# 2Retr0/GodotOceanWaves

Hardware: AMD Instinct MI355X
Metric: displacement+normal maps/sec, 1024^2 x 4 cascades; achieved HBM GB/s vs peak (higher is better)
Workload: dtype f32; 1 GPU; 1024^2 x 4 cascades per GPU, steady-state tick (modulate + 2-D IFFT + unpack/foam), delta=1/50 s, SURVEY 8d cascade table; map_size=1024, cascades_per_gpu=4, parallelism=cascade-sharded x1, gather=none

## Files before the change

### godotoceanwaves_amd/csrc/ow_device.h

```cpp
#pragma once

#include <stdint.h>
#include <math.h>

#if defined(__HIPCC__)
#define OW_DEV __device__ __forceinline__
#define OW_HD __host__ __device__ __forceinline__
#define OW_DEVICE_BUILD 1
#define OW_SCHED_FENCE() __builtin_amdgcn_sched_barrier(0)
#else
#define OW_DEV inline
#define OW_HD inline
#define OW_DEVICE_BUILD 0
#define OW_SCHED_FENCE() ((void)0)
#endif

namespace ow {

#if OW_DEVICE_BUILD
typedef float cplx __attribute__((ext_vector_type(2)));
#else
struct alignas(8) cplx {
    float x, y;
};
// ... 457 lines not shown
    float f;
    __builtin_memcpy(&f, &x, 4);
    return f;
#endif
}
OW_DEV uint32_t f2h2(float lo, float hi) {
#if OW_DEVICE_BUILD && OW_CVT_PK
    uint32_t r;
    asm("v_cvt_pk_f16_f32 %0, %1, %2" : "=v"(r) : "v"(lo), "v"(hi));
    return r;
#else
    return (uint32_t)f2h(lo) | ((uint32_t)f2h(hi) << 16);
#endif
}

struct CascadeFrame {
    float tile_x, tile_y;
    float time;
    float whitecap;
    float foam_grow_rate;
    float foam_decay;
    int32_t cascade;
    int32_t fault;
};
constexpr uint32_t kStatusRowSyncTimeout = 1u;
constexpr unsigned long long kRowSyncTimeoutTicks = 2000000ull;
constexpr int plan_lp_rows(int N) { return 128 / plan_T(N) > 0 ? 128 / plan_T(N) : 1; }
constexpr int plan_lp_threads(int N) { return plan_lp_rows(N) * kLayers * plan_T(N); }
constexpr int plan_lp_lds_cplx(int N) { return plan_region_cplx(N) * plan_lp_rows(N) * kLayers + plan_tw_total(N); }
constexpr int plan_lp_handoff_cplx(int N) { return plan_lp_threads(N) / 2; }

template <int N>
struct TickPlan {
    static constexpr int Q = plan_lp_threads(N) / plan_wg_threads(N);
    static constexpr int GPS = N / kWgRows;
    static_assert(Q >= 1 && plan_lp_threads(N) % plan_wg_threads(N) == 0 && (GPS / 2) % Q == 0, "block shapes of the two passes must nest");
    static constexpr int full(int slots) { return slots * GPS / Q; }
    static constexpr int upper(int slots) { return slots * (GPS / 2) / Q; }
    static constexpr int row0(int slots) { return (slots * 3 + Q - 1) / Q; }
    static constexpr int items_1(int slots) { return 2 * full(slots) + upper(slots) + row0(slots); }
    static constexpr int items_1_compact(int slots) { return full(slots); }
    static OW_HD void decode_compact(int item, int sub, int &slot, int &row0) {
        const int group = item * Q + sub;
        slot = group / GPS;
        row0 = (group % GPS) * kWgRows;
    }
    static constexpr int items_2(int slots) { return slots * (N / plan_lp_rows(N)); }
    static constexpr int kPipeRows = plan_lp_rows(N) / 2 > 0 ? plan_lp_rows(N) / 2 : 1;
    static constexpr int items_2_pipe(int slots) { return slots * (N / kPipeRows); }
    static OW_HD bool decode(int item, int sub, int slots, int &L, int &slot, int &row0) {
        const int n_full = full(slots), n_upper = upper(slots);
        if (item < 2 * n_full) {
            L = item < n_full ? 0 : 2;
            const int group = (item < n_full ? item : item - n_full) * Q + sub;
            slot = group / GPS;
            row0 = (group % GPS) * kWgRows;
            return true;
        }
        if (item < 2 * n_full + n_upper) {
            L = 1;
            const int group = (item - 2 * n_full) * Q + sub;
            slot = group / (GPS / 2);
            row0 = N / 2 + (group % (GPS / 2)) * kWgRows;
            return true;
        }
        const int r = (item - 2 * n_full - n_upper) * Q + sub;
        const bool active = r < slots * 3;
        slot = active ? r / 3 : 0;
        L = 3 + (active ? r % 3 : 0);
        row0 = 0;
        return active;
    }
};

constexpr int kMaxTickGroup = 16;
struct TickGroupArgs {
    float time1[kMaxTickGroup][8];
    int32_t tbase2[kMaxTickGroup];
    int32_t tbase1[kMaxTickGroup];
    int32_t slots, n2, n1, d2, d1;
    int32_t pair_compact;
    int32_t first2, slots2;
    int32_t first1, slots1;
    int32_t step1;
    int32_t p2_pipe;
    int32_t p1_compact;
};
struct PairFrame {
    float tile_x, tile_y, whitecap, foam_grow_rate, foam_decay;
    int32_t cascade;
};
struct PairArgs {
    PairFrame c[8];
    float time1[8];
    int32_t tbase2, tbase1;
    int32_t n2, n1;
    int32_t first2, first1;
    int32_t fault, pad;
};
OW_HD CascadeFrame pair_frame(const PairArgs &g, int launch_slot) {
    const PairFrame &f = g.c[launch_slot];
    CascadeFrame cf;
    cf.tile_x = f.tile_x, cf.tile_y = f.tile_y, cf.time = g.time1[launch_slot], cf.whitecap = f.whitecap;
    cf.foam_grow_rate = f.foam_grow_rate, cf.foam_decay = f.foam_decay, cf.cascade = f.cascade, cf.fault = g.fault;
    return cf;
}
constexpr int32_t kFaultRowSync = 1;
constexpr int kMaxCascades = 8;
struct FrameArgs {
    CascadeFrame c[kMaxCascades];
};

#if OW_DEVICE_BUILD
typedef uint32_t u32x4_t __attribute__((ext_vector_type(4)));
typedef uint32_t u32x2_t __attribute__((ext_vector_type(2)));
struct GBuf {
    __amdgpu_buffer_rsrc_t r;
};
OW_DEV GBuf make_gbuf(const void *base, uint32_t bytes) {
    return GBuf{__builtin_amdgcn_make_buffer_rsrc(const_cast<void *>(base), 0, (int)bytes, 0x00020000)};
}
template <int AUX = 0>
OW_DEV f32x4 gload16(GBuf b, uint32_t voff, uint32_t soff) {
    return __builtin_bit_cast(f32x4, __builtin_amdgcn_raw_buffer_load_b128(b.r, (int)voff, (int)soff, AUX));
}
template <int AUX = 0>
OW_DEV cplx gload8(GBuf b, uint32_t voff, uint32_t soff) {
    return __builtin_bit_cast(cplx, __builtin_amdgcn_raw_buffer_load_b64(b.r, (int)voff, (int)soff, AUX));
}
template <int AUX = 0>
OW_DEV float gload4(GBuf b, uint32_t voff, uint32_t soff) {
    return __builtin_bit_cast(float, __builtin_amdgcn_raw_buffer_load_b32(b.r, (int)voff, (int)soff, AUX));
}
template <int AUX = 0>
OW_DEV uint16_t gload2(GBuf b, uint32_t voff, uint32_t soff) {
    return (uint16_t)__builtin_amdgcn_raw_buffer_load_b16(b.r, (int)voff, (int)soff, AUX);
}
template <int AUX = 0>
OW_DEV void gstore8(GBuf b, uint32_t voff, uint32_t soff, cplx v) {
    __builtin_amdgcn_raw_buffer_store_b64(__builtin_bit_cast(u32x2_t, v), b.r, (int)voff, (int)soff, AUX);
}
template <int AUX = 0>
OW_DEV void gstore8h(GBuf b, uint32_t voff, uint32_t soff, u16x4 v) {
    __builtin_amdgcn_raw_buffer_store_b64(__builtin_bit_cast(u32x2_t, v), b.r, (int)voff, (int)soff, AUX);
}
template <int AUX = 0>
OW_DEV void gstore8w(GBuf b, uint32_t voff, uint32_t soff, uint32_t w0, uint32_t w1) {
    __builtin_amdgcn_raw_buffer_store_b64(u32x2_t{w0, w1}, b.r, (int)voff, (int)soff, AUX);
}
template <int AUX = 0>
OW_DEV void gstore16(GBuf b, uint32_t voff, uint32_t soff, f32x4 v) {
    __builtin_amdgcn_raw_buffer_store_b128(__builtin_bit_cast(u32x4_t, v), b.r, (int)voff, (int)soff, AUX);
}
#else
struct GBuf {
    char *p;
};
OW_DEV GBuf make_gbuf(const void *base, uint32_t) { return GBuf{(char *)const_cast<void *>(base)}; }
template <int AUX = 0>
OW_DEV f32x4 gload16(GBuf b, uint32_t voff, uint32_t soff) { f32x4 v; __builtin_memcpy(&v, b.p + voff + soff, 16); return v; }
template <int AUX = 0>
OW_DEV cplx gload8(GBuf b, uint32_t voff, uint32_t soff) { cplx v; __builtin_memcpy(&v, b.p + voff + soff, 8); return v; }
template <int AUX = 0>
OW_DEV float gload4(GBuf b, uint32_t voff, uint32_t soff) { float v; __builtin_memcpy(&v, b.p + voff + soff, 4); return v; }
template <int AUX = 0>
OW_DEV uint16_t gload2(GBuf b, uint32_t voff, uint32_t soff) { uint16_t v; __builtin_memcpy(&v, b.p + voff + soff, 2); return v; }
template <int AUX = 0>
OW_DEV void gstore8(GBuf b, uint32_t voff, uint32_t soff, cplx v) { __builtin_memcpy(b.p + voff + soff, &v, 8); }
template <int AUX = 0>
OW_DEV void gstore8h(GBuf b, uint32_t voff, uint32_t soff, u16x4 v) { __builtin_memcpy(b.p + voff + soff, &v, 8); }
template <int AUX = 0>
OW_DEV void gstore8w(GBuf b, uint32_t voff, uint32_t soff, uint32_t w0, uint32_t w1) {
    const uint32_t w[2] = {w0, w1};
    __builtin_memcpy(b.p + voff + soff, w, 8);
}
template <int AUX = 0>
OW_DEV void gstore16(GBuf b, uint32_t voff, uint32_t soff, f32x4 v) { __builtin_memcpy(b.p + voff + soff, &v, 16); }
#endif
constexpr int kAuxDefault = 0, kAuxNT = 2, kAuxAgent = 16;

OW_HD constexpr uint32_t t_unit(int n, int layer, int xp, int y) {
    return ((((uint32_t)layer * (uint32_t)(n >> 4) + (uint32_t)(y >> 4)) * (uint32_t)n + (uint32_t)xp) << 4) + (uint32_t)(y & 15);
}
constexpr uint32_t t_cascade_bytes(int n) { return (uint32_t)n * (uint32_t)n * kLayers * 8u; }

OW_DEV float modulate_kcomp(int id, int n, float tile) {
    return ((((float)id - (float)n * 0.5f) * 2.0f) * kPi) / tile;
}

#ifndef OW_OMEGA_ONE_LOAD
#define OW_OMEGA_ONE_LOAD 1
#endif
template <int N>
struct Pass1 {
    static constexpr int T = plan_T(N), P = kP;

    static constexpr int rot(int j) { return (j + 8) & 15; }

    template <int AUX = 0, int J0 = 0, int J1 = P>
    static OW_DEV void load_raw(cplx *a, cplx *b, float *om, int t, int y, GBuf h0_c, GBuf om_c) {
        const int ym = (N - y) % N;
        const int tm = (T - t) % T;
        const uint32_t a_off = (uint32_t)(y * N + t) * 8u;
        const uint32_t b_off = (uint32_t)(ym * N + tm) * 8u;
        const bool lane0 = (t == 0);
        const bool om_mirror = y > N / 2;
        const uint32_t o_off = (om_mirror ? (uint32_t)(ym * N + tm) : (uint32_t)(y * N + t)) * 4u;
#pragma unroll
        for (int j = J0; j < J1; ++j) {
            const int blk = rot(j);
            a[j] = gload8<AUX>(h0_c, a_off, (uint32_t)(T * blk) * 8u);
            const uint32_t mb = (uint32_t)(T * (15 - blk)), mb0 = (uint32_t)(T * ((16 - blk) % 16));
            constexpr bool one_load = OW_OMEGA_ONE_LOAD && T >= 64;
            if (blk == 0) {
                b[j] = gload8<AUX>(h0_c, lane0 ? b_off : b_off + mb * 8u, 0u);
                if constexpr (one_load) om[j] = gload4<AUX>(om_c, (om_mirror && !lane0) ? o_off + mb * 4u : o_off, 0u);
                else om[j] = om_mirror ? gload4<AUX>(om_c, lane0 ? o_off : o_off + mb * 4u, 0u) : gload4<AUX>(om_c, o_off, 0u);
            } else {
                b[j] = gload8<AUX>(h0_c, lane0 ? b_off + (uint32_t)T * 8u : b_off, mb * 8u);
                (void)mb0;
                if constexpr (one_load) {
#if OW_DEVICE_BUILD
                    const bool mirror_u = __builtin_amdgcn_readfirstlane((int)om_mirror) != 0;
#else
                    const bool mirror_u = om_mirror;
#endif
                    om[j] = gload4<AUX>(om_c, (om_mirror && lane0) ? o_off + (uint32_t)T * 4u : o_off, mirror_u ? mb * 4u : (uint32_t)(T * blk) * 4u);
                } else {
                    om[j] = om_mirror ? gload4<AUX>(om_c, lane0 ? o_off + (uint32_t)T * 4u : o_off, mb * 4u)
                                      : gload4<AUX>(om_c, o_off, (uint32_t)(T * blk) * 4u);
                }
            }
        }
    }
    static constexpr bool kPairwise = N >= 1024;
#ifndef OW_P1_PAIRWISE
#define OW_P1_PAIRWISE 7
#endif
    template <int J0 = 0, int J1 = P>
    static OW_DEV void modulate(cplx *h, const cplx *a, const cplx *b, const float *om, float time) {
        static_assert(J0 % 2 == 0 && J1 % 2 == 0, "texels are modulated two at a time");
#if OW_DEVICE_BUILD && (OW_P1_PAIRWISE & 1)
        if constexpr (kPairwise) {
#pragma unroll
            for (int j = J0; j < J1; j += 2) {
                const cplx ph = cplx{om[j], om[j + 1]} * cplx{time, time};
                const cplx q = ph * cplx{0.318309886183790672f, 0.318309886183790672f};
                const cplx n = cplx{__builtin_rintf(q.x), __builtin_rintf(q.y)};
                cplx r = __builtin_elementwise_fma(-n, cplx{3.140625f, 3.140625f}, ph);
                r = __builtin_elementwise_fma(-n, cplx{9.67502593994140625e-4f, 9.67502593994140625e-4f}, r);
                r = __builtin_elementwise_fma(-n, cplx{1.509957990978376432e-7f, 1.509957990978376432e-7f}, r);
                const cplx z = r * r;
                cplx ps = cplx{2.6343420813645935e-06f, 2.6343420813645935e-06f};
                ps = __builtin_elementwise_fma(ps, z, cplx{-0.00019822614558506757f, -0.00019822614558506757f});
                ps = __builtin_elementwise_fma(ps, z, cplx{0.008333241567015648f, 0.008333241567015648f});
                ps = __builtin_elementwise_fma(ps, z, cplx{-0.1666666567325592f, -0.1666666567325592f});
                const cplx sn = __builtin_elementwise_fma(ps * z, r, r);
                cplx pc = cplx{-2.654252000411361e-07f, -2.654252000411361e-07f};
                pc = __builtin_elementwise_fma(pc, z, cplx{2.478597525623627e-05f, 2.478597525623627e-05f});
                pc = __builtin_elementwise_fma(pc, z, cplx{-0.0013888811226934195f, -0.0013888811226934195f});
                pc = __builtin_elementwise_fma(pc, z, cplx{0.0416666679084301f, 0.0416666679084301f});
                const cplx cs = __builtin_elementwise_fma(pc * z, z, __builtin_elementwise_fma(cplx{-0.5f, -0.5f}, z, cplx{1.0f, 1.0f}));
#pragma unroll
                for (int e = 0; e < 2; ++e) {
                    const uint32_t flip = (uint32_t)(int)(e ? n.y : n.x) << 31;
                    const float se = e ? sn.y : sn.x, ce = e ? cs.y : cs.x;
                    const float s = __builtin_bit_cast(float, __builtin_bit_cast(uint32_t, se) ^ flip);
                    const float c = __builtin_bit_cast(float, __builtin_bit_cast(uint32_t, ce) ^ flip);
                    const cplx pp = cadd(a[j + e], b[j + e]), qq = csub(a[j + e], b[j + e]);
                    h[j + e] = cplx{__builtin_fmaf(pp.x, c, -mul_rn(pp.y, s)), __builtin_fmaf(qq.y, c, mul_rn(qq.x, s))};
                    opaque_inplace(h[j + e]);
                }
                if (j % 4 == 2) OW_SCHED_FENCE();
            }
            return;
        }
#endif
#pragma unroll
        for (int j = J0; j < J1; ++j) {
            const cplx m = expi_phase(mul_rn(om[j], time));
            const cplx pp = cadd(a[j], b[j]), qq = csub(a[j], b[j]);
#if OW_DEVICE_BUILD
            const cplx t1 = pp * m, t2 = qq * m.yx;
#else
            const cplx t1 = cplx{pp.x * m.x, pp.y * m.y}, t2 = cplx{qq.x * m.y, qq.y * m.x};
#endif
            h[j] = cplx{t1.x - t1.y, t2.x + t2.y};
            opaque_inplace(h[j]);
            if (j % 4 == 3) OW_SCHED_FENCE();
        }
    }
    template <int AUX = 0>
    static OW_DEV void load_modulate(cplx *h, int t, int y, GBuf h0_c, GBuf om_c, float time) {
        cplx a[P], b[P];
        float om[P];
        load_raw<AUX>(a, b, om, t, y, h0_c, om_c);
        modulate(h, a, b, om, time);
    }

    static OW_DEV float kx_of(int j, float kx0, float dkx) { return __builtin_fmaf((float)(T * rot(j)), dkx, kx0); }
    static OW_DEV void wave_numbers(float *ik, int t, float ky, float dkx) {
        const float kx0 = (float)(t - N / 2) * dkx, ky2 = __builtin_fmaf(ky, ky, 1e-30f);
#if OW_DEVICE_BUILD && (OW_P1_PAIRWISE & 2)
        if constexpr (kPairwise) {
#pragma unroll
            for (int j = 0; j < P; j += 2) {
// ... 97 lines not shown
    }
    template <int Q>
    static OW_DEV void row0_input(cplx *d, const cplx *h, const float *ik, int t, float ky, float dkx) {
        const float kx0 = (float)(t - N / 2) * dkx;
#pragma unroll
        for (int j = 0; j < P; ++j) {
            const cplx ih = cmuli(h[j]);
            const float kx = kx_of(j, kx0, dkx), ux = kx * ik[j], uy = ky * ik[j];
            const bool corner = (j == kColSlot) && (t == 0);
            float a = 0.0f, b = 0.0f;
            if (Q == 1) { a = corner ? kx - ky * uy : -(ky * uy); b = corner ? ux : 0.0f; }
            if (Q == 2) { a = -ky; b = corner ? -(ky * ux) : ux; }
            if (Q == 3) { a = corner ? 0.0f : ky * ux; b = corner ? -(kx * ux) : __builtin_fmaf(-kx, ux, kx); }
            d[j] = cadd(cscale(h[j], a), cscale(ih, b));
            opaque_inplace(d[j]);
            if (j % 4 == 3) OW_SCHED_FENCE();
        }
    }

    static OW_DEV void stage_write(const cplx *d, int t, cplx *lds_row) {
#pragma unroll
        for (int o = 0; o < P; ++o) lds_row[t + T * o] = d[OutMap<N>::slot_of(o)];
    }
    template <int AUX>
    static OW_DEV void stage_store(int tau, int layer, int row0, const cplx *lds_block, GBuf T_c) {
        const int q = tau % kWgRows, xi = tau / kWgRows;
        const cplx *st = lds_block + q * plan_region_cplx(N);
        const uint32_t voff = t_unit(N, 0, xi, row0 + q) * 8u;
        cplx v[P];
#pragma unroll
        for (int k = 0; k < P; ++k) v[k] = lds_read(st + xi + T * k);
#pragma unroll
        for (int k = 0; k < P; ++k) gstore8<AUX>(T_c, voff, (t_unit(N, layer, 0, 0) + t_unit(N, 0, T * k, 0)) * 8u, v[k]);
    }
    template <int AUX>
    static OW_DEV void stage_store_chunk(int tau, int layer, int row0, const cplx *lds_block, GBuf T_c, int g) {
        const int q = tau % kWgRows, xi = tau / kWgRows;
        const cplx *st = lds_block + q * plan_region_cplx(N);
        const uint32_t voff = t_unit(N, 0, xi, row0 + q) * 8u;
        cplx v[4];
#pragma unroll
        for (int k = 0; k < 4; ++k) v[k] = lds_read(st + xi + T * (4 * g + k));
#pragma unroll
        for (int k = 0; k < 4; ++k) gstore8<AUX>(T_c, voff, (t_unit(N, layer, 0, 0) + t_unit(N, 0, T * (4 * g + k), 0)) * 8u, v[k]);
    }
};

template <int N>
struct Pass2 {
    static constexpr int T = plan_T(N), P = kP;

    static OW_DEV uint32_t t_voff(int t, int xp) {
        return (T >= 16 ? t_unit(N, 0, xp, t) : t_unit(N, 0, xp, 0) + (uint32_t)t) * 8u;
    }
    static constexpr uint32_t t_soff(int layer, int j) {
        return (t_unit(N, layer, 0, 0) + (T >= 16 ? t_unit(N, 0, 0, T * j) : t_unit(N, 0, 0, 16 * (j / 2)) + 8u * (j % 2))) * 8u;
    }
    static constexpr int rot(int j) { return (j + 8) & 15; }
    template <int AUX>
    static OW_DEV void load_layer(cplx *d, int t, int xp, int layer, GBuf T_c) {
        const uint32_t voff = t_voff(t, xp);
#pragma unroll
        for (int j = 0; j < P; ++j) d[j] = gload8<AUX>(T_c, voff, t_soff(layer, rot(j)));
    }
    OW_HD static constexpr uint32_t foam_index(int xp, int yp) { return (uint32_t)xp * N + (uint32_t)(yp % T) * 16u + (uint32_t)(yp / T); }
    static OW_DEV void load_foam(uint32_t *pk, int t, int xp, GBuf foam_c) {
        const uint32_t voff = foam_index(xp, t) * 2u;
        const f32x4 a = gload16(foam_c, voff, 0u), b = gload16(foam_c, voff, 16u);
        const float v[8] = {a.x, a.y, a.z, a.w, b.x, b.y, b.z, b.w};
#pragma unroll
        for (int i = 0; i < 8; ++i) pk[i] = __builtin_bit_cast(uint32_t, v[i]);
    }
    static OW_DEV void store_foam(const uint32_t *pk, int t, int xp, GBuf foam_c) {
        const uint32_t voff = foam_index(xp, t) * 2u;
        float v[8];
#pragma unroll
        for (int i = 0; i < 8; ++i) v[i] = __builtin_bit_cast(float, pk[i]);
        gstore16(foam_c, voff, 0u, f32x4{v[0], v[1], v[2], v[3]});
        gstore16(foam_c, voff, 16u, f32x4{v[4], v[5], v[6], v[7]});
    }

    static OW_DEV void f32_put(GBuf f32_c, uint32_t tex, int o, int ch, float v) {
#if OW_DEVICE_BUILD
        __builtin_amdgcn_raw_buffer_store_b32(__builtin_bit_cast(uint32_t, v), f32_c.r, (int)(tex * 32u + (uint32_t)ch * 4u), (int)((uint32_t)(T * o) * 32u), 0);
#else
        __builtin_memcpy(f32_c.p + tex * 32u + (uint32_t)ch * 4u + (uint32_t)(T * o) * 32u, &v, 4);
#endif
    }

    template <bool F32>
    static OW_DEV void after_layer3(const cplx *l3, const cplx *l2, uint32_t *foam_pk, uint32_t *gy_foam,
                                    uint32_t tex, const CascadeFrame &cf, GBuf f32_c) {
#pragma unroll
        for (int o = 0; o < P; ++o) {
            const int sl = OutMap<N>::slot_of(o);
            const float dhy_dz = l2[sl].x, dhx_dx = l2[sl].y;
            const float dhz_dz = l3[sl].x, dhz_dx = l3[sl].y;
            const float jac = (1.0f + dhx_dx) * (1.0f + dhz_dz) - dhz_dx * dhz_dx;
            const float foam_factor = -fminf(0.0f, jac - cf.whitecap);
            float foam = h2f((uint16_t)((foam_pk[o / 2] >> (16 * (o & 1))) & 0xFFFFu));
            foam = mul_rn(foam, cf.foam_decay);
            foam = foam + mul_rn(foam_factor, cf.foam_grow_rate);
            foam = fminf(fmaxf(foam, 0.0f), 1.0f);
            const float gy = dhy_dz * fast_rcp(1.0f + fabsf(dhz_dz));
            const uint32_t foam_h = f2h(foam);
            gy_foam[o] = (uint32_t)f2h(gy) | (foam_h << 16);
            foam_pk[o / 2] = (o & 1) ? ((foam_pk[o / 2] & 0xFFFFu) | (foam_h << 16)) : ((foam_pk[o / 2] & 0xFFFF0000u) | foam_h);
            if (F32) {
                f32_put(f32_c, tex, o, 4, gy);
                f32_put(f32_c, tex, o, 6, foam);
                f32_put(f32_c, tex, o, 7, jac);
            }
        }
    }
    template <bool F32, int AUX>
    static OW_DEV void after_layer1(const cplx *l1, const float *dhx_dx, const uint32_t *gy_foam, uint32_t tex, GBuf norm_c,
                                    GBuf f32_c) {
#pragma unroll
        for (int o = 0; o < P; ++o) {
            const int sl = OutMap<N>::slot_of(o);
            const float gx = l1[sl].y * fast_rcp(1.0f + fabsf(dhx_dx[o]));
            gstore8h<AUX>(norm_c, tex * 8u, (uint32_t)(T * o) * 8u,
                          u16x4{f2h(gx), (uint16_t)(gy_foam[o] & 0xFFFFu), f2h(dhx_dx[o]), (uint16_t)(gy_foam[o] >> 16)});
            if (F32) {
                f32_put(f32_c, tex, o, 3, gx);
                f32_put(f32_c, tex, o, 5, dhx_dx[o]);
            }
        }
    }
    static constexpr int kRow0Slot = 8;
    static OW_DEV float ky_of(int j, int t, float dky) { return (float)(t + T * (rot(j) - 8)) * dky; }
    OW_HD static constexpr uint32_t pcol_index(int y) { return (uint32_t)(y % T) * 16u + (uint32_t)(y / T); }
    template <int AUX = 0>
    static OW_DEV void derive_dx(cplx *d, int t, int xp, float dky, GBuf pcol_c) {
        const float s = (xp & 1) ? -1.0f : 1.0f;
#pragma unroll
        for (int half = 0; half < 2; ++half) {
            cplx p[P / 2];
#pragma unroll
            for (int i = 0; i < P / 4; ++i) {
                const f32x4 v = gload16<AUX>(pcol_c, (uint32_t)t * 128u, 16u * (uint32_t)(i + (P / 4) * (1 - half)));
                p[2 * i] = cplx{v.x, v.y};
                p[2 * i + 1] = cplx{v.z, v.w};
            }
#pragma unroll
            for (int k = 0; k < P / 2; ++k) {
                const int j = 8 * half + k;
                const float ky = ky_of(j, t, dky);
                d[j] = cplx{__builtin_fmaf(-ky, d[j].y, s * p[k].x), __builtin_fmaf(ky, d[j].x, s * p[k].y)};
            }
            OW_SCHED_FENCE();
        }
    }
    template <int AUX>
    static OW_DEV void load_c1(cplx *d, int t, int xp, float dky, GBuf T_c) {
        static_assert(T >= 16, "the mirrored offsets below assume that T is a multiple of the 16-row line");
        const uint32_t voff = t_voff(t, xp);
        const uint32_t voff_m = t_unit(N, 0, xp, N - t - 7 * T) * 8u;
        const float kyb = (float)t * dky;
        cplx v[P];
#pragma unroll
        for (int j = 0; j < P; ++j)
            v[j] = j < P / 2 ? gload8<AUX>(T_c, voff, t_soff(1, rot(j))) : gload8<AUX>(T_c, voff_m, (t_unit(N, 1, 0, 0) + t_unit(N, 0, 0, T * (15 - j))) * 8u);
        OW_SCHED_FENCE();
#pragma unroll
        for (int j = 0; j < P; ++j) {
            const float sc = 1.0f - __builtin_fmaf((float)(T * (rot(j) - 8)), dky, kyb);
            d[j] = j < P / 2 ? cscale(v[j], sc) : cplx{v[j].x * sc, v[j].y * -sc};
        }
    }
    static OW_DEV void put_row0(cplx *d, int t, cplx r) {
        d[kRow0Slot] = cplx{t == 0 ? r.x : d[kRow0Slot].x, t == 0 ? r.y : d[kRow0Slot].y};
    }
    template <bool F32>
    static OW_DEV void after_f2(const cplx *f2, uint32_t *hz_pk, float *c2, uint32_t tex, GBuf f32_c) {
#pragma unroll
        for (int o = 0; o < P; o += 2) {
            const int sl = OutMap<N>::slot_of(o), sl1 = OutMap<N>::slot_of(o + 1);
            c2[o] = f2[sl].y * f2[sl].y;
            c2[o + 1] = f2[sl1].y * f2[sl1].y;
            hz_pk[o / 2] = (uint32_t)opaque((int)f2h2(f2[sl].x, f2[sl1].x));
            if (F32) {
                f32_put(f32_c, tex, o, 2, f2[sl].x);
                f32_put(f32_c, tex, o + 1, 2, f2[sl1].x);
            }
        }
    }
    template <bool F32, int AUX>
    static OW_DEV void after_f0(const cplx *f0, const uint32_t *hz_pk, int t, int xp, uint32_t tex, GBuf disp_c, GBuf f32_c) {
        const uint32_t w = (uint32_t)((xp ^ t) & 1) << 31;
#pragma unroll
        for (int o = 0; o < P; ++o) {
            const int sl = OutMap<N>::slot_of(o);
            const uint32_t hz_h = (hz_pk[o / 2] >> (16 * (o & 1))) & 0xFFFFu;
            gstore8w<AUX>(disp_c, tex * 8u, (uint32_t)(T * o) * 8u, f2h2(f0[sl].x, f0[sl].y), hz_h | w);
            if (F32) {
                f32_put(f32_c, tex, o, 0, f0[sl].x);
                f32_put(f32_c, tex, o, 1, f0[sl].y);
            }
        }
    }
    template <bool F32>
    static OW_DEV void after_f1(const cplx *f1, float *dhx_dx, uint32_t *gx_pk, uint32_t tex, GBuf f32_c) {
#pragma unroll
        for (int o = 0; o < P; o += 2) {
            const int sl = OutMap<N>::slot_of(o), sl1 = OutMap<N>::slot_of(o + 1);
            dhx_dx[o] = f1[sl].x;
            dhx_dx[o + 1] = f1[sl1].x;
            const float gx = f1[sl].y * fast_rcp(1.0f + fabsf(dhx_dx[o])), gx1 = f1[sl1].y * fast_rcp(1.0f + fabsf(dhx_dx[o + 1]));
            gx_pk[o / 2] = (uint32_t)opaque((int)f2h2(gx, gx1));
            if (F32) {
                f32_put(f32_c, tex, o, 3, gx);
                f32_put(f32_c, tex, o, 5, dhx_dx[o]);
                f32_put(f32_c, tex, o + 1, 3, gx1);
                f32_put(f32_c, tex, o + 1, 5, dhx_dx[o + 1]);
            }
        }
    }
    template <bool F32, int AUX>
    static OW_DEV void after_f3(const cplx *f3, const float *dhx_dx, const float *c2, const uint32_t *gx_pk, uint32_t *foam_pk,
                                uint32_t tex, const CascadeFrame &cf, GBuf norm_c, GBuf f32_c) {
#pragma unroll
        for (int o = 0; o < P; o += 2) {
            float foam[2], gy[2];
#pragma unroll
            for (int e = 0; e < 2; ++e) {
                const int sl = OutMap<N>::slot_of(o + e);
                const float dhy_dz = f3[sl].x, dhz_dz = f3[sl].y;
                const float jac = (1.0f + dhx_dx[o + e]) * (1.0f + dhz_dz) - c2[o + e];
                const float foam_factor = -fminf(0.0f, jac - cf.whitecap);
                float fm = h2f((uint16_t)((foam_pk[o / 2] >> (16 * e)) & 0xFFFFu));
                fm = mul_rn(fm, cf.foam_decay);
                fm = fm + mul_rn(foam_factor, cf.foam_grow_rate);
                foam[e] = fminf(fmaxf(fm, 0.0f), 1.0f);
                gy[e] = dhy_dz * fast_rcp(1.0f + fabsf(dhz_dz));
                if (F32) {
                    f32_put(f32_c, tex, o + e, 4, gy[e]);
                    f32_put(f32_c, tex, o + e, 6, foam[e]);
                    f32_put(f32_c, tex, o + e, 7, jac);
                }
            }
            foam_pk[o / 2] = f2h2(foam[0], foam[1]);
            const uint32_t gy_pk = f2h2(gy[0], gy[1]), gxw = gx_pk[o / 2];
            gstore8w<AUX>(norm_c, tex * 8u, (uint32_t)(T * o) * 8u, (gxw & 0xFFFFu) | (gy_pk << 16), f2h2(dhx_dx[o], foam[0]));
            gstore8w<AUX>(norm_c, tex * 8u, (uint32_t)(T * (o + 1)) * 8u, (gxw >> 16) | (gy_pk & 0xFFFF0000u), f2h2(dhx_dx[o + 1], foam[1]));
        }
    }

    template <bool F32, int AUX>
    static OW_DEV uint16_t unpack_texel(cplx l0, cplx l1, cplx l2, cplx l3, uint16_t foam_prev, int t, int xp, int o, uint32_t tex,
                                        const CascadeFrame &cf, GBuf disp_c, GBuf norm_c, GBuf f32_c) {
        const float dhy_dz = l2.x, dhx_dx = l2.y, dhz_dz = l3.x, dhz_dx = l3.y;
        const float jac = (1.0f + dhx_dx) * (1.0f + dhz_dz) - dhz_dx * dhz_dx;
        const float foam_factor = -fminf(0.0f, jac - cf.whitecap);
        float foam = h2f(foam_prev);
        foam = mul_rn(foam, cf.foam_decay);
        foam = foam + mul_rn(foam_factor, cf.foam_grow_rate);
        foam = fminf(fmaxf(foam, 0.0f), 1.0f);
        const float gy = dhy_dz * fast_rcp(1.0f + fabsf(dhz_dz));
        const float gx = l1.y * fast_rcp(1.0f + fabsf(dhx_dx));
        const uint32_t n1 = f2h2(dhx_dx, foam);
        const uint16_t foam_h = (uint16_t)(n1 >> 16);
        const uint32_t w = (uint32_t)((xp ^ t) & 1) << 31;
        gstore8w<AUX>(norm_c, tex * 8u, (uint32_t)(T * o) * 8u, f2h2(gx, gy), n1);
        gstore8w<AUX>(disp_c, tex * 8u, (uint32_t)(T * o) * 8u, f2h2(l0.x, l0.y), (uint32_t)f2h(l1.x) | w);
        if (F32) {
            f32_put(f32_c, tex, o, 0, l0.x);
            f32_put(f32_c, tex, o, 1, l0.y);
            f32_put(f32_c, tex, o, 2, l1.x);
            f32_put(f32_c, tex, o, 3, gx);
            f32_put(f32_c, tex, o, 4, gy);
            f32_put(f32_c, tex, o, 5, dhx_dx);
            f32_put(f32_c, tex, o, 6, foam);
            f32_put(f32_c, tex, o, 7, jac);
        }
        return foam_h;
    }

    template <bool F32, int AUX>
    static OW_DEV void after_layer0(const cplx *l0, const float *hz, int t, int xp, uint32_t tex, GBuf disp_c, GBuf f32_c) {
        const uint16_t w = (uint16_t)(((xp ^ t) & 1) << 15);
#pragma unroll
        for (int o = 0; o < P; ++o) {
            const int sl = OutMap<N>::slot_of(o);
            gstore8h<AUX>(disp_c, tex * 8u, (uint32_t)(T * o) * 8u, u16x4{f2h(l0[sl].x), f2h(l0[sl].y), f2h(hz[o]), w});
            if (F32) {
                f32_put(f32_c, tex, o, 0, l0[sl].x);
                f32_put(f32_c, tex, o, 1, l0[sl].y);
                f32_put(f32_c, tex, o, 2, hz[o]);
            }
        }
    }
};

struct SpectrumPC {
    int32_t seed_x, seed_y;
    float tile_x, tile_y;
    float alpha, peak_frequency, wind_speed, angle, depth, swell, detail, spread;
};

OW_DEV float omega_texel(int x, int y, int n, float tile_x, float tile_y, float depth) {
#if defined(__clang__)
#pragma clang fp contract(off)
#endif
    const float kx = modulate_kcomp(x, n, tile_x), ky = modulate_kcomp(y, n, tile_y);
    const float k = sqrtf(kx * kx + ky * ky) + 1e-6f;
    const float a = k * depth;
    const float b = a > 9.1f ? 1.0f : (float)tanh((double)a);
    return sqrtf(kG * k * b);
}

OW_DEV void hash_uniform(uint32_t x, uint32_t y, float &u1, float &u2) {
    uint32_t h32 = y + 374761393u + x * 3266489917u;
    h32 = 2246822519u * (h32 ^ (h32 >> 15));
    h32 = 3266489917u * (h32 ^ (h32 >> 13));
    const uint32_t n = h32 ^ (h32 >> 16), n2 = n * 48271u;
    const float rden = 1.0f / 2147483648.0f;
    u1 = (float)((n >> 1) & 0x7FFFFFFFu) * rden;
    u2 = (float)((n2 >> 1) & 0x7FFFFFFFu) * rden;
}

OW_DEV cplx spectrum_amplitude(int idx, int idy, int n, const SpectrumPC &pc) {
#if defined(__clang__)
#pragma clang fp contract(off)
#endif
    const float dkx = (2.0f * kPi) / pc.tile_x, dky = (2.0f * kPi) / pc.tile_y;
// ... 99 lines not shown
```

### godotoceanwaves_amd/csrc/ow_frame_kernels.h

```cpp
#pragma once
#include <type_traits>

#include "ow_kernels.h"

#ifndef OW_P1_WAVES
#define OW_P1_WAVES 4
#endif
namespace ow {

struct Stamp {
    unsigned long long t[16];
    unsigned xcc, pad;
    unsigned long long rt0, rt1;
};
struct DebugArgs {
    Stamp *stamps;
    int never_true;
};

__device__ __forceinline__ void wave_sync() {
    __builtin_amdgcn_fence(__ATOMIC_RELEASE, "wavefront");
    __builtin_amdgcn_wave_barrier();
    __builtin_amdgcn_fence(__ATOMIC_ACQUIRE, "wavefront");
}
// ... 409 lines not shown
    }
    {
        cplx l0[P];
        fetch(l0, 0);
        if constexpr (kFft) row_ifft<N>(l0, t, lds_row, tw_lds, rs);
        OW_STAMP(3, l0[0].x)
        if (kStore || dbg.never_true) {
            Pass2<N>::template after_layer0<F32, AUX_O>(l0, hz, t, xp, tex, disp_c, f32_c);
        } else {
#pragma unroll
            for (int j = 0; j < P; ++j) keep += l0[j].x + l0[j].y + hz[j];
        }
    }
    if (!kStore && keep == 12345.678f) buf.disp[t] = u16x4{1, 2, 3, 4};
    if constexpr ((VAR & 8) != 0) {
        asm volatile("s_waitcnt vmcnt(0)" ::: "memory");
        ts[14] = __builtin_readcyclecounter();
        write_stamps<(plan_wg_threads(N) + 63) / 64>(ts, dbg);
    }
}


template <int N, int AUX_T, int AUX_H, class Issued, class Stamper>
__device__ __forceinline__ void pass1c_item(const DeviceBuffers &buf, const CascadeFrame &cf, float time, int tslot, int row0, int tau, cplx *tw_lds,
                                            cplx *rows_lds, RowSync<N> &rs, Issued issued, Stamper stamp) {
    constexpr int Tn = plan_T(N), P = kP, LC = Pass1<N>::kCompactLayers;
    const int rw = (Tn >= 64) ? __builtin_amdgcn_readfirstlane(tau / Tn) : tau / Tn, t = tau % Tn;
    const uint32_t plane = (uint32_t)N * N;
    cplx *lds_row = rows_lds + rw * plan_region_cplx(N);
    const int y = row0 + rw;
    const GBuf h0_c = make_gbuf(buf.h0 + (size_t)cf.cascade * plane, plane * 8u);
    const GBuf om_c = make_gbuf(buf.omega + (size_t)cf.cascade * plane, plane * 4u);
    const GBuf T_c = make_gbuf(buf.T + (size_t)tslot * plane * kLayers, t_cascade_bytes(N));
    const GBuf pcol_c = make_gbuf(buf.pcol + (size_t)tslot * N, (uint32_t)N * 8u);
    const GBuf rrow_c = make_gbuf(buf.rrow + (size_t)tslot * N * 4, (uint32_t)N * 32u);

    cplx h[P];
    const float dkx = (2.0f * kPi) / cf.tile_x, dky = (2.0f * kPi) / cf.tile_y;
    const float ky = (float)(y - N / 2) * dky;
    float ik[P];
    {
        cplx a[P], b[P];
        float om[P];
        Pass1<N>::template load_raw<AUX_H>(a, b, om, t, y, h0_c, om_c);
        issued();
        Pass1<N>::modulate(h, a, b, om, time);
    }
    stamp(1, h[0].x);
    Pass1<N>::wave_numbers(ik, t, ky, dkx);
    if (t == 0) gstore8(pcol_c, Pass2<N>::pcol_index(y) * 8u, 0u, Pass1<N>::column_term(h, ik, t, dkx));

    if (__builtin_amdgcn_readfirstlane(y) == 0) {
#pragma unroll
        for (int Q = 1; Q <= 3; ++Q) {
            cplx d[P];
            OW_SCHED_FENCE();
            {
                const float kyo = opaque(ky), dkxo = opaque(dkx);
                const int to = opaque(t);
#pragma unroll
                for (int j = 0; j < P; ++j) opaque_inplace(h[j]);
                if (Q == 1) Pass1<N>::template row0_input<1>(d, h, ik, to, kyo, dkxo);
                if (Q == 2) Pass1<N>::template row0_input<2>(d, h, ik, to, kyo, dkxo);
                if (Q == 3) Pass1<N>::template row0_input<3>(d, h, ik, to, kyo, dkxo);
            }
            OW_SCHED_FENCE();
            row_ifft<N, false>(d, t, lds_row, tw_lds, rs);
            rs.sync();
            if (y == 0) {
#pragma unroll
                for (int o = 0; o < P; ++o) gstore8(rrow_c, (uint32_t)(t + Tn * o) * 32u, (uint32_t)Q * 8u, d[OutMap<N>::slot_of(o)]);
            }
        }
    }

    const bool lower = row0 < N / 2;
#pragma unroll
    for (int L = 0; L < LC; ++L) {
        if (L == 1 && lower) continue;
        cplx d[P];
        OW_SCHED_FENCE();
        {
            const float kyo = opaque(ky), dkxo = opaque(dkx);
            const int to = opaque(t);
#pragma unroll
            for (int j = 0; j < P; ++j) opaque_inplace(h[j]);
            auto drain = [&](int g) {
                if (L > 0) Pass1<N>::template stage_store_chunk<AUX_T>(tau, (L == 2 && lower) ? 0 : L - 1, row0, rows_lds, T_c, g);
            };
            if (L == 0) Pass1<N>::template layer_input_c<0>(d, h, ik, to, kyo, dkxo, drain);
            if (L == 1) Pass1<N>::template layer_input_c<1>(d, h, ik, to, kyo, dkxo, drain);
            if (L == 2) Pass1<N>::template layer_input_c<2>(d, h, ik, to, kyo, dkxo, drain);
        }
        OW_SCHED_FENCE();
        stamp(2 + 3 * L, d[0].x);
        if (L > 0) row_ifft<N, true>(d, t, lds_row, tw_lds, rs);
        else row_ifft<N, false>(d, t, lds_row, tw_lds, rs);
        stamp(3 + 3 * L, d[0].x);
        rs.sync();
        Pass1<N>::stage_write(d, t, lds_row);
        lds_barrier();
        if (L == LC - 1) Pass1<N>::template stage_store<AUX_T>(tau, L, row0, rows_lds, T_c);
        stamp(4 + 3 * L, d[0].x);
    }
}

template <int N, int AUX_T = kAuxDefault, int AUX_H = kAuxDefault, bool STAMPS = false>
__global__ __launch_bounds__(plan_wg_threads(N), OW_P1_WAVES) void k_pass1c(DeviceBuffers buf, FrameArgs args, Stamp *stamps = nullptr) {
    unsigned long long ts[STAMPS ? 16 : 1] = {0};
    auto stamp = [&](int k, float keep) {
        if constexpr (STAMPS) {
            asm volatile("" ::"v"(keep));
            ts[k] = __builtin_readcyclecounter();
        }
    };
    stamp(0, 0.0f);
    constexpr int Tn = plan_T(N);
    static_assert(Tn >= 16, "Pass2::load_c1 needs N/16 to be a multiple of the 16-row line");
    __shared__ __attribute__((aligned(16))) cplx lds[plan_wg_lds_cplx(N) + plan_sync_flag_cplx(N, kWgRows)];
    cplx *tw_lds = lds;
    cplx *rows_lds = lds + plan_tw_total(N);
    const int tau = threadIdx.x;
    int *sync_flags = reinterpret_cast<int *>(lds + plan_wg_lds_cplx(N));
    RowSync<N> rs;
    rs.attach(sync_flags, tau / Tn, (tau / 64) & 1);
    rs.watch(buf.status, args.c[0].fault);
    init_row_sync<N>(sync_flags, kWgRows);

    int slot, row0;
    p1_block_to_rows<N>(slot, row0);
    const CascadeFrame cf = args.c[slot];
    fetch_arguments(buf, cf);
    TwPrefetch<N> twp;
    tw_fetch<N>(twp, buf.tw);
    pass1c_item<N, AUX_T, AUX_H>(buf, cf, cf.time, slot, row0, tau, tw_lds, rows_lds, rs, [&] { tw_commit<N>(twp, tw_lds); }, stamp);
    if constexpr (STAMPS) {
        asm volatile("s_waitcnt vmcnt(0)" ::: "memory");
        ts[14] = __builtin_readcyclecounter();
        ts[15] = (unsigned long long)row0;
        if ((threadIdx.x & 63) == 0) {
            Stamp st;
            for (int k = 0; k < 16; ++k) st.t[k] = ts[k];
            st.xcc = xcc_id();
            st.pad = 0;
            stamps[blockIdx.x * ((plan_wg_threads(N) + 63) / 64) + threadIdx.x / 64] = st;
        }
    }
}

constexpr bool p2c_half_table(int N) { return plan_row_spans_waves(N); }
constexpr int p2c_table_total(int N) { return p2c_half_table(N) ? plan_twh_total(N) : plan_tw_total(N); }
template <int N>
__device__ __forceinline__ const cplx *p2c_table(const DeviceBuffers &buf) { return p2c_half_table(N) ? buf.tw_half : buf.tw; }
template <int N, bool F32, int AUX_T, int AUX_O, class RS, class Issued>
__device__ __forceinline__ void pass2c_item(const DeviceBuffers &buf, const CascadeFrame &cf, int tslot, int row0, int tau, cplx *tw_lds, cplx *rows_lds,
                                            RS &rs, Issued issued, uint32_t (&foam_pk)[kP / 2], int foam_io = 3) {
    constexpr int Tn = plan_T(N), P = kP;
    constexpr bool TWH = p2c_half_table(N);
    const int rw = (Tn >= 64) ? __builtin_amdgcn_readfirstlane(tau / Tn) : tau / Tn, t = tau % Tn;
    const uint32_t plane = (uint32_t)N * N;
    cplx *lds_row = rows_lds + rw * plan_region_cplx(N);
    const int xp = row0 + rw;
    const GBuf T_c = make_gbuf(buf.T + (size_t)tslot * plane * kLayers, t_cascade_bytes(N));
    const GBuf pcol_c = make_gbuf(buf.pcol + (size_t)tslot * N, (uint32_t)N * 8u);
    const GBuf rrow_c = make_gbuf(buf.rrow + (size_t)tslot * N * 4, (uint32_t)N * 32u);
    const GBuf disp_c = make_gbuf(buf.disp + (size_t)cf.cascade * plane, plane * 8u);
    const GBuf norm_c = make_gbuf(buf.norm + (size_t)cf.cascade * plane, plane * 8u);
    const GBuf foam_c = make_gbuf(buf.foam + (size_t)cf.cascade * plane, plane * 2u);
    const GBuf f32_c = make_gbuf(F32 ? buf.f32 + (size_t)cf.cascade * plane * 8 : nullptr, F32 ? plane * 32u : 0u);
    const float dky = (2.0f * kPi) / cf.tile_y;
    auto side_row = [&](int q) { return gload8(rrow_c, (uint32_t)xp * 32u, (uint32_t)q * 8u); };

    uint32_t hz_pk[P / 2];
    float c2[P];
    {
        cplx f2[P];
        OW_SCHED_FENCE();
        Pass2<N>::template load_c1<AUX_T>(f2, t, xp, dky, T_c);
        const cplx r2 = side_row(2);
        issued();
        Pass2<N>::put_row0(f2, t, r2);
        row_ifft<N, false, TWH>(f2, opaque(t), lds_row, tw_lds, rs);
        OW_SCHED_FENCE();
        Pass2<N>::template after_f2<F32>(f2, hz_pk, c2, (uint32_t)(xp * N + opaque(t)), f32_c);
    }
    cplx c0[P];
    {
        cplx f0[P];
        OW_SCHED_FENCE();
        const int tq = opaque(t);
        Pass2<N>::template load_layer<AUX_T>(c0, tq, xp, 0, T_c);
#pragma unroll
        for (int j = 0; j < P; ++j) f0[j] = c0[j];
        row_ifft<N, false, TWH>(f0, opaque(t), lds_row, tw_lds, rs);
        OW_SCHED_FENCE();
        const int tr = opaque(t);
        Pass2<N>::template after_f0<F32, AUX_O>(f0, hz_pk, tr, xp, (uint32_t)(xp * N + tr), disp_c, f32_c);
    }
    float dhx_dx[P];
    uint32_t gx_pk[P / 2];
    {
        OW_SCHED_FENCE();
        const int tq = opaque(t);
        Pass2<N>::derive_dx(c0, tq, xp, dky, pcol_c);
        Pass2<N>::put_row0(c0, tq, side_row(1));
        row_ifft<N, false, TWH>(c0, opaque(t), lds_row, tw_lds, rs);
        OW_SCHED_FENCE();
        Pass2<N>::template after_f1<F32>(c0, dhx_dx, gx_pk, (uint32_t)(xp * N + opaque(t)), f32_c);
    }
    {
        cplx f3[P];
        OW_SCHED_FENCE();
        const int tq = opaque(t);
        Pass2<N>::template load_layer<AUX_T>(f3, tq, xp, 2, T_c);
        Pass2<N>::put_row0(f3, tq, side_row(3));
        if (foam_io & 1) Pass2<N>::load_foam(foam_pk, tq, xp, foam_c);
        row_ifft<N, false, TWH>(f3, opaque(t), lds_row, tw_lds, rs);
        OW_SCHED_FENCE();
        const int tr = opaque(t);
        Pass2<N>::template after_f3<F32, AUX_O>(f3, dhx_dx, c2, gx_pk, foam_pk, (uint32_t)(xp * N + tr), cf, norm_c, f32_c);
        if (foam_io & 2) Pass2<N>::store_foam(foam_pk, tr, xp, foam_c);
    }
}

template <int N, bool F32, int AUX_T = kAuxDefault, int AUX_O = kAuxDefault>
__global__ __launch_bounds__(plan_wg_threads(N), 4) void k_pass2c(DeviceBuffers buf, FrameArgs args) {
    constexpr int Tn = plan_T(N);
    static_assert(Tn >= 16, "Pass2::load_c1 needs N/16 to be a multiple of the 16-row line");
    constexpr int TW = p2c_table_total(N), ROWS_CPLX = plan_region_cplx(N) * kWgRows;
    __shared__ __attribute__((aligned(16))) cplx lds[TW + ROWS_CPLX + plan_sync_flag_cplx(N, kWgRows)];
    cplx *tw_lds = lds;
    cplx *rows_lds = lds + TW;
    const int tau = threadIdx.x;
    int *sync_flags = reinterpret_cast<int *>(lds + TW + ROWS_CPLX);
    RowSync<N> rs;
    rs.attach(sync_flags, tau / Tn, (tau / 64) & 1);
    rs.watch(buf.status, args.c[0].fault);
    init_row_sync<N>(sync_flags, kWgRows);

    int slot, row0;
    p2_block_to_rows<N>(slot, row0);
    const CascadeFrame cf = args.c[slot];
    fetch_arguments(buf, cf);
    TablePrefetch<TW, plan_wg_threads(N)> twp;
    twp.fetch(p2c_table<N>(buf));
    uint32_t foam_pk[kP / 2];
    pass2c_item<N, F32, AUX_T, AUX_O>(buf, cf, slot, row0, tau, tw_lds, rows_lds, rs, [&] { twp.commit(tw_lds); }, foam_pk);
}

#ifndef OW_SPLIT_P1_ROWS
#define OW_SPLIT_P1_ROWS 4
#endif
template <int N, int ROWS = kWgRows>
struct SplitGeo {
    static constexpr int H = N / 2, TH = plan_T(H), R = plan_region_cplx(H), TW = plan_tw_total(H);
    static constexpr int kRows = ROWS;
    static constexpr int kThreads = 2 * ROWS * TH;
    static constexpr int kLdsCplx = TW + 2 * ROWS * R;
    static constexpr int kTwPerThread = (TW + kThreads - 1) / kThreads;
};
template <class SG>
struct SplitTw {
    cplx v[SG::kTwPerThread];
};
template <class SG>
__device__ __forceinline__ void split_tw_fetch(SplitTw<SG> &p, const cplx *__restrict__ tw_split, int tau) {
#pragma unroll
    for (int k = 0; k < SG::kTwPerThread; ++k) {
        const int i = tau + k * SG::kThreads;
        p.v[k] = tw_split[i < SG::TW ? i : 0];
    }
}
template <class SG>
__device__ __forceinline__ void split_tw_commit(const SplitTw<SG> &p, cplx *tw_lds, int tau) {
#pragma unroll
    for (int k = 0; k < SG::kTwPerThread; ++k) {
        const int i = tau + k * SG::kThreads;
        if (i < SG::TW) tw_lds[i] = p.v[k];
    }
    lds_barrier();
}

template <int N, int ROWS, int AUX_T, int AUX_H, class Stamper>
__device__ __forceinline__ void pass1c_split_item(const DeviceBuffers &buf, const CascadeFrame &cf, float time, int tslot, int row0, int fault, cplx *tw_lds,
                                                  cplx *rows_lds, int *sync_flags, int tau, Stamper stamp) {
    using SG = SplitGeo<N, ROWS>;
    constexpr int H = SG::H, TH = SG::TH, P = kP, LC = Pass1<N>::kCompactLayers, T = plan_T(N);
    const int wv = __builtin_amdgcn_readfirstlane(tau / 64), rw = wv >> 1, w = wv & 1;
    const int tp = tau % 64, t = 2 * tp + w;
    cplx *vrow = rows_lds + (w * ROWS + rw) * SG::R;
    const uint32_t plane = (uint32_t)N * N;
    RowSync<H> rs;
    RowSync<N> pair;
    pair.attach(sync_flags, rw, w);
    pair.watch(buf.status, fault);
    if (tau < 2 * ROWS) sync_flags[tau] = 0;

    const int y = row0 + rw;
    const GBuf h0_c = make_gbuf(buf.h0 + (size_t)cf.cascade * plane, plane * 8u);
    const GBuf om_c = make_gbuf(buf.omega + (size_t)cf.cascade * plane, plane * 4u);
    const GBuf T_c = make_gbuf(buf.T + (size_t)tslot * plane * kLayers, t_cascade_bytes(N));
    const GBuf pcol_c = make_gbuf(buf.pcol + (size_t)tslot * N, (uint32_t)N * 8u);
    const GBuf rrow_c = make_gbuf(buf.rrow + (size_t)tslot * N * 4, (uint32_t)N * 32u);

    const int q = tau % ROWS, xi = tau / ROWS;
    cplx h[P];
    cplx wxi;
    const float dkx = (2.0f * kPi) / cf.tile_x, dky = (2.0f * kPi) / cf.tile_y;
    const float ky = (float)(y - N / 2) * dky;
    float ik[P];
    {
        SplitTw<SG> twv;
        split_tw_fetch<SG>(twv, buf.tw_split, tau);
        wxi = buf.tw_split[SG::TW + xi];
        cplx a[P], b[P];
        float om[P];
        Pass1<N>::template load_raw<AUX_H>(a, b, om, t, y, h0_c, om_c);
        stamp(1, 0.0f);
        split_tw_commit<SG>(twv, tw_lds, tau);
        stamp(2, a[15].x + om[15]);
        Pass1<N>::modulate(h, a, b, om, time);
    }
    stamp(3, h[15].x);
    Pass1<N>::wave_numbers(ik, t, ky, dkx);
    if (t == 0) gstore8(pcol_c, Pass2<N>::pcol_index(y) * 8u, 0u, Pass1<N>::column_term(h, ik, t, dkx));

    const cplx *e_reg = rows_lds + q * SG::R, *o_reg = rows_lds + (ROWS + q) * SG::R;
    auto combine = [&](int m, cplx &lo, cplx &hi) {
        const cplx e = lds_read(e_reg + xi + T * m), o = lds_read(o_reg + xi + T * m);
        cplx wx = wxi;
        opaque_inplace(wx);
        cplx tw = wx;
        switch (m) {
            case 1: tw = cmul_const(wx, root32_cos(2), root32_sin(2)); break;
            case 2: tw = cmul_const(wx, root32_cos(4), root32_sin(4)); break;
            case 3: tw = cmul_const(wx, root32_cos(6), root32_sin(6)); break;
            case 4: tw = cmuli(wx); break;
            case 5: tw = cmul_const(wx, root32_cos(10), root32_sin(10)); break;
            case 6: tw = cmul_const(wx, root32_cos(12), root32_sin(12)); break;
            case 7: tw = cmul_const(wx, root32_cos(14), root32_sin(14)); break;
            default: break;
        }
        const cplx z = cmul(o, tw);
        lo = cadd(e, z);
        hi = csub(e, z);
    };
    const uint32_t voff = t_unit(N, 0, xi, row0 + q) * 8u;
    auto store_chunk = [&](int layer, int g) {
#pragma unroll
        for (int mm = 0; mm < 2; ++mm) {
            const int m = 2 * g + mm;
            cplx lo, hi;
            combine(m, lo, hi);
            gstore8<AUX_T>(T_c, voff, (t_unit(N, layer, 0, 0) + t_unit(N, 0, T * m, 0)) * 8u, lo);
            gstore8<AUX_T>(T_c, voff, (t_unit(N, layer, 0, 0) + t_unit(N, 0, T * (m + 8), 0)) * 8u, hi);
            OW_SCHED_FENCE();
        }
    };

    if (__builtin_amdgcn_readfirstlane(y) == 0) {
        const int xr = tp + TH * w;
        const cplx wxr = buf.tw_split[SG::TW + xr];
        const cplx *e0 = rows_lds + rw * SG::R, *o0 = rows_lds + (ROWS + rw) * SG::R;
#pragma unroll
        for (int Q = 1; Q <= 3; ++Q) {
            cplx d[P];
            OW_SCHED_FENCE();
            {
                const float kyo = opaque(ky), dkxo = opaque(dkx);
// ... 593 lines not shown
```

Measured before the change: 82690 maps/s.

## Hoist side-row and pcol loads earlier in pass2c to overlap latency

```diff
diff --git a/godotoceanwaves_amd/csrc/ow_device.h b/godotoceanwaves_amd/csrc/ow_device.h
--- a/godotoceanwaves_amd/csrc/ow_device.h
+++ b/godotoceanwaves_amd/csrc/ow_device.h
@@ -633,6 +633,11 @@
 OW_DEV void gstore16(GBuf b, uint32_t voff, uint32_t soff, f32x4 v) {
     __builtin_amdgcn_raw_buffer_store_b128(__builtin_bit_cast(u32x4_t, v), b.r, (int)voff, (int)soff, AUX);
 }
+typedef float f32x8_t __attribute__((ext_vector_type(8)));
+OW_DEV f32x8_t sload32(const void *p) {
+    typedef const __attribute__((address_space(4))) f32x8_t *const_ptr;
+    return *(const_ptr)(uintptr_t)p;
+}
 #else
 struct GBuf {
     char *p;
@@ -1036,6 +1041,26 @@
             OW_SCHED_FENCE();
         }
     }
+    template <int AUX = 0>
+    static OW_DEV void pcol_issue(f32x4 *pv, int half, int t, GBuf pcol_c) {
+#pragma unroll
+        for (int i = 0; i < P / 4; ++i) pv[(P / 4) * half + i] = gload16<AUX>(pcol_c, (uint32_t)t * 128u, 16u * (uint32_t)(i + (P / 4) * (1 - half)));
+    }
+    static OW_DEV void derive_dx_from(cplx *d, const f32x4 *pv, int t, int xp, float dky) {
+        const float s = (xp & 1) ? -1.0f : 1.0f;
+#pragma unroll
+        for (int half = 0; half < 2; ++half) {
+#pragma unroll
+            for (int k = 0; k < P / 2; ++k) {
+                const int j = 8 * half + k;
+                const f32x4 v = pv[(P / 4) * half + k / 2];
+                const cplx p = (k & 1) ? cplx{v.z, v.w} : cplx{v.x, v.y};
+                const float ky = ky_of(j, t, dky);
+                d[j] = cplx{__builtin_fmaf(-ky, d[j].y, s * p.x), __builtin_fmaf(ky, d[j].x, s * p.y)};
+            }
+            OW_SCHED_FENCE();
+        }
+    }
     template <int AUX>
     static OW_DEV void load_c1(cplx *d, int t, int xp, float dky, GBuf T_c) {
         static_assert(T >= 16, "the mirrored offsets below assume that T is a multiple of the 16-row line");
@@ -1056,6 +1081,14 @@
     static OW_DEV void put_row0(cplx *d, int t, cplx r) {
         d[kRow0Slot] = cplx{t == 0 ? r.x : d[kRow0Slot].x, t == 0 ? r.y : d[kRow0Slot].y};
     }
+#if OW_DEVICE_BUILD
+    static OW_DEV void put_row0_lane0(cplx *d, cplx r) {
+        float x = d[kRow0Slot].x, y = d[kRow0Slot].y;
+        asm("v_writelane_b32 %0, %1, 0" : "+v"(x) : "s"(r.x));
+        asm("v_writelane_b32 %0, %1, 0" : "+v"(y) : "s"(r.y));
+        d[kRow0Slot] = cplx{x, y};
+    }
+#endif
     template <bool F32>
     static OW_DEV void after_f2(const cplx *f2, uint32_t *hz_pk, float *c2, uint32_t tex, GBuf f32_c) {
 #pragma unroll
diff --git a/godotoceanwaves_amd/csrc/ow_frame_kernels.h b/godotoceanwaves_amd/csrc/ow_frame_kernels.h
--- a/godotoceanwaves_amd/csrc/ow_frame_kernels.h
+++ b/godotoceanwaves_amd/csrc/ow_frame_kernels.h
@@ -585,11 +585,17 @@
 constexpr int p2c_table_total(int N) { return p2c_half_table(N) ? plan_twh_total(N) : plan_tw_total(N); }
 template <int N>
 __device__ __forceinline__ const cplx *p2c_table(const DeviceBuffers &buf) { return p2c_half_table(N) ? buf.tw_half : buf.tw; }
+#ifndef OW_P2_EARLY
+#define OW_P2_EARLY 1
+#endif
 template <int N, bool F32, int AUX_T, int AUX_O, class RS, class Issued>
 __device__ __forceinline__ void pass2c_item(const DeviceBuffers &buf, const CascadeFrame &cf, int tslot, int row0, int tau, cplx *tw_lds, cplx *rows_lds,
                                             RS &rs, Issued issued, uint32_t (&foam_pk)[kP / 2], int foam_io = 3) {
     constexpr int Tn = plan_T(N), P = kP;
     constexpr bool TWH = p2c_half_table(N);
+    constexpr int EARLY = (F32 && Tn < 64) ? 0 : (Tn < 64) ? (OW_P2_EARLY & 7) : OW_P2_EARLY;
+    constexpr bool SIDE_EARLY = (EARLY & 1) != 0, SIDE_SCALAR = SIDE_EARLY && Tn >= 64;
+    constexpr bool PCOL_EARLY = (EARLY & 2) != 0, C0_EARLY = (EARLY & 4) != 0, C2_EARLY = (EARLY & 8) != 0;
     const int rw = (Tn >= 64) ? __builtin_amdgcn_readfirstlane(tau / Tn) : tau / Tn, t = tau % Tn;
     const uint32_t plane = (uint32_t)N * N;
     cplx *lds_row = rows_lds + rw * plan_region_cplx(N);
@@ -603,51 +609,95 @@
     const GBuf f32_c = make_gbuf(F32 ? buf.f32 + (size_t)cf.cascade * plane * 8 : nullptr, F32 ? plane * 32u : 0u);
     const float dky = (2.0f * kPi) / cf.tile_y;
     auto side_row = [&](int q) { return gload8(rrow_c, (uint32_t)xp * 32u, (uint32_t)q * 8u); };
+    cplx r1, r2, r3;
+    if constexpr (SIDE_SCALAR) {
+        const f32x8_t rec = sload32(buf.rrow + ((size_t)tslot * N + (size_t)xp) * 4);
+        r1 = cplx{rec[2], rec[3]};
+        r2 = cplx{rec[4], rec[5]};
+        r3 = cplx{rec[6], rec[7]};
+    }
+    auto put_row0 = [&](cplx *d, int tq, cplx r) {
+        if constexpr (SIDE_SCALAR) {
+            if (Tn == 64 || __builtin_amdgcn_readfirstlane(t) == 0) Pass2<N>::put_row0_lane0(d, r);
+        } else {
+            Pass2<N>::put_row0(d, tq, r);
+        }
+    };
 
     uint32_t hz_pk[P / 2];
     float c2[P];
+    cplx c0[P];
     {
         cplx f2[P];
         OW_SCHED_FENCE();
+        if constexpr (SIDE_EARLY && !SIDE_SCALAR) {
+            r1 = side_row(1);
+            r2 = side_row(2);
+            r3 = side_row(3);
+        }
         Pass2<N>::template load_c1<AUX_T>(f2, t, xp, dky, T_c);
-        const cplx r2 = side_row(2);
+        if constexpr (!SIDE_EARLY) r2 = side_row(2);
         issued();
-        Pass2<N>::put_row0(f2, t, r2);
+        put_row0(f2, t, r2);
         row_ifft<N, false, TWH>(f2, opaque(t), lds_row, tw_lds, rs);
         OW_SCHED_FENCE();
+        if constexpr (C0_EARLY) {
+            Pass2<N>::template load_layer<AUX_T>(c0, opaque(t), xp, 0, T_c);
+            OW_SCHED_FENCE();
+        }
         Pass2<N>::template after_f2<F32>(f2, hz_pk, c2, (uint32_t)(xp * N + opaque(t)), f32_c);
     }
-    cplx c0[P];
+    f32x4 pv[P / 2];
     {
         cplx f0[P];
         OW_SCHED_FENCE();
         const int tq = opaque(t);
-        Pass2<N>::template load_layer<AUX_T>(c0, tq, xp, 0, T_c);
+        if constexpr (!C0_EARLY) Pass2<N>::template load_layer<AUX_T>(c0, tq, xp, 0, T_c);
 #pragma unroll
         for (int j = 0; j < P; ++j) f0[j] = c0[j];
         row_ifft<N, false, TWH>(f0, opaque(t), lds_row, tw_lds, rs);
         OW_SCHED_FENCE();
         const int tr = opaque(t);
+        if constexpr (PCOL_EARLY) {
+            Pass2<N>::pcol_issue(pv, 0, tr, pcol_c);
+            OW_SCHED_FENCE();
+        }
         Pass2<N>::template after_f0<F32, AUX_O>(f0, hz_pk, tr, xp, (uint32_t)(xp * N + tr), disp_c, f32_c);
     }
     float dhx_dx[P];
     uint32_t gx_pk[P / 2];
+    cplx f3[P];
     {
         OW_SCHED_FENCE();
         const int tq = opaque(t);
-        Pass2<N>::derive_dx(c0, tq, xp, dky, pcol_c);
-        Pass2<N>::put_row0(c0, tq, side_row(1));
+        if constexpr (PCOL_EARLY) {
+            Pass2<N>::pcol_issue(pv, 1, tq, pcol_c);
+            OW_SCHED_FENCE();
+            Pass2<N>::derive_dx_from(c0, pv, tq, xp, dky);
+        } else {
+            Pass2<N>::derive_dx(c0, tq, xp, dky, pcol_c);
+        }
+        if constexpr (!SIDE_EARLY) r1 = side_row(1);
+        put_row0(c0, tq, r1);
         row_ifft<N, false, TWH>(c0, opaque(t), lds_row, tw_lds, rs);
         OW_SCHED_FENCE();
+        if constexpr (C2_EARLY) {
+            const int tr = opaque(t);
+            Pass2<N>::template load_layer<AUX_T>(f3, tr, xp, 2, T_c);
+            if (foam_io & 1) Pass2<N>::load_foam(foam_pk, tr, xp, foam_c);
+            OW_SCHED_FENCE();
+        }
         Pass2<N>::template after_f1<F32>(c0, dhx_dx, gx_pk, (uint32_t)(xp * N + opaque(t)), f32_c);
     }
     {
-        cplx f3[P];
         OW_SCHED_FENCE();
         const int tq = opaque(t);
-        Pass2<N>::template load_layer<AUX_T>(f3, tq, xp, 2, T_c);
-        Pass2<N>::put_row0(f3, tq, side_row(3));
-        if (foam_io & 1) Pass2<N>::load_foam(foam_pk, tq, xp, foam_c);
+        if constexpr (!C2_EARLY) Pass2<N>::template load_layer<AUX_T>(f3, tq, xp, 2, T_c);
+        if constexpr (!SIDE_EARLY) r3 = side_row(3);
+        put_row0(f3, tq, r3);
+        if constexpr (!C2_EARLY) {
+            if (foam_io & 1) Pass2<N>::load_foam(foam_pk, tq, xp, foam_c);
+        }
         row_ifft<N, false, TWH>(f3, opaque(t), lds_row, tw_lds, rs);
         OW_SCHED_FENCE();
         const int tr = opaque(t);
```

Result: faster. 83610 maps/s, median of 6 (+1.1%).
